# camillabelponer/dealii-slod

Measured on NVIDIA B200. Metric: slod_basis_patches_per_s, higher is better.
Workload: dtype f64

## Files before the change

dealii-slod_b200/csrc/capi.cu:

```cuda
#include <cuda_runtime.h>
#include <dlfcn.h>
#include <nccl.h>

#include <algorithm>
#include <array>
#include <cmath>
#include <cstdio>
#include <cstdlib>
#include <cstring>
#include <mutex>
#include <numeric>
#include <string>
#include <thread>
#include <vector>

#include "../../include/slod.h"
#include "geom.h"
#include "kernels.h"

using namespace slod;

namespace {

std::string g_create_error;

struct Timings {
  double ms[8] = {0, 0, 0, 0, 0, 0, 0, 0};
};

}

struct slod_ctx {
  slod_params par{};
  Params P{};
  int device = 0;
  int n_sm = 148;
  int64_t n_patches = 0;
  int n_fields = 1;
  bool coef_set[2] = {false, false};
  std::vector<double> coef_table[2];
  int coef_r[2] = {0, 0};
  bool coef_dirty = true;
  double *d_coef = nullptr;
  size_t d_coef_elems = 0;
  size_t coef_field_elems = 0;
  double *d_phi = nullptr, *d_aphi = nullptr, *d_Kell = nullptr, *d_diag = nullptr;
  int *d_status = nullptr;
  int *d_counter = nullptr;
  int *d_work_counter = nullptr;
  bool basis_done = false, coarse_done = false;
  int chunk = 0;
  bool chunk_limited = false;
  int64_t ids_cap = 0;
  int *d_ids = nullptr;
  double *d_X = nullptr, *d_Minv = nullptr, *d_G = nullptr, *d_cvec = nullptr, *d_Lws = nullptr, *d_W = nullptr, *d_coefws = nullptr;
  FluxLayout xl{};
  size_t smem_flux = 0;
  int grid_flux = 0;
  int solve_grid = 0;
  int dense_ntile = 0;
  int mma_variant = -1;
  bool dense_coef_gmem = false;
  int mma_threads = 0;
  int mma_nip = 0, mma_stw = 0;
  bool split_solver = false;
  size_t smem_factor = 0, smem_tri = 0;
  double *d_Lrec = nullptr;
  double *d_stw = nullptr;
  cudaEvent_t ev_split = nullptr;
  float split_factor_ms = 0;
  long long mma_lws_per_cta = 0;
  SolveLayout sl{};
  DenseLayout dl{};
  SelectPlan sp{};
  SelectBuffers sb{};
  FinishLayout fl{};
  size_t smem_solve = 0, smem_dense = 0, smem_finish = 0, smem_coarse = 0, smem_coarse_blk = 0;
  int coarse_nu = 0;
  int grid_solve = 0, grid_dense = 0, grid_finish = 0, grid_coarse = 0;
  int bw_max = 0, nb_max = 0;
  cudaEvent_t ev[12]{};
  std::vector<cudaEvent_t> chunk_ev;
  size_t chunks_pending = 0;
  bool basis_pending = false;
  int64_t pending_p0 = 0, pending_p1 = 0;
  int *h_status = nullptr;
  Timings tm;
  int64_t launches = 0;
  std::vector<int> ids;
  int64_t ids_p0 = -1, ids_p1 = -1;
  mutable std::string err;
  mutable std::vector<int64_t> fine_numbering;
  bool csr_ready = false;
  std::vector<int64_t> csr_rowptr, csr_col;
  long long *d_perm = nullptr;
  cudaStream_t copy_stream = nullptr;
  bool coarse_timing_pending = false;
  double *d_online = nullptr;
  size_t online_doubles = 0;
  double *d_batch = nullptr;
  size_t batch_doubles = 0;
  double *d_val = nullptr;
  int64_t csr_nnz = 0;
  double *d_Mell = nullptr, *d_Mval = nullptr, *d_Sell = nullptr;
  bool mass_done = false;
  double s_dt = 0.0;
  double *d_heat = nullptr;
  size_t heat_doubles = 0;
  std::vector<slod_ctx *> subs;
  ncclComm_t comm = nullptr;
  int comm_rank = 0, comm_world = 1;
// ... 432 lines not shown
  if (ctx->ids_p0 != p0 || ctx->ids_p1 != p1) {
    std::vector<int> order((size_t)(p1 - p0));
    std::iota(order.begin(), order.end(), (int)p0);
    std::vector<long long> cost(order.size());
    for (size_t i = 0; i < order.size(); ++i) {
      const Geom g = make_geom(P, order[i]);
      cost[i] = (long long)g.Ni * g.bw * (g.bw + 4LL * g.Ncd) + (long long)g.Ncd * g.Ncd * g.Ncd * 8;
    }
    std::vector<int> perm(order.size());
    std::iota(perm.begin(), perm.end(), 0);
    std::stable_sort(perm.begin(), perm.end(), [&](int a, int b) { return cost[a] > cost[b]; });
    ctx->ids.resize(order.size());
    for (size_t i = 0; i < perm.size(); ++i) ctx->ids[i] = order[perm[i]];
    CK(cudaMemcpyAsync(ctx->d_ids, ctx->ids.data(), sizeof(int) * ctx->ids.size(), cudaMemcpyHostToDevice, st));
    CK(cudaStreamSynchronize(st));
    ctx->ids_p0 = p0;
    ctx->ids_p1 = p1;
  }
  const size_t n_ids = ctx->ids.size();
  if (!ctx->h_status) CK(cudaHostAlloc(&ctx->h_status, sizeof(int) * (size_t)ctx->n_patches, cudaHostAllocDefault));
  CK(cudaMemsetAsync(ctx->d_status + p0, 0, sizeof(int) * (size_t)(p1 - p0), st));

  static const bool static_stride = getenv("SLOD_STATIC_WORK") != nullptr;
  int *wc = static_stride ? nullptr : ctx->d_work_counter;
  const size_t n_chunks = (n_ids + ctx->chunk - 1) / ctx->chunk;
  while (ctx->chunk_ev.size() < 5 * n_chunks) {
    cudaEvent_t e;
    CK(cudaEventCreate(&e));
    ctx->chunk_ev.push_back(e);
  }
  ctx->chunks_pending = 0;
  for (size_t off = 0, ci = 0; off < n_ids; off += ctx->chunk, ++ci) {
    const int nw = (int)std::min<size_t>(ctx->chunk, n_ids - off);
    const int *ids = ctx->d_ids + off;
    cudaEvent_t *ev = ctx->chunk_ev.data() + 5 * ci;
    CK(cudaEventRecord(ev[0], st));
    if (ctx->split_solver) {
      static const int factor_grid_env = getenv("SLOD_FACTOR_GRID") ? atoi(getenv("SLOD_FACTOR_GRID")) : 0;
      CK(launch_patch_factor(std::min(nw, factor_grid_env > 0 ? factor_grid_env : 2 * ctx->n_sm), ctx->smem_factor, st, ids, nw, ctx->d_coef, ctx->d_Lrec,
                             ctx->d_stw, ctx->d_status, ctx->sl.coef_doubles, ctx->mma_nip, ctx->sl.ldx, ctx->sl.x_stride, wc));
      if (ci == 0) CK(cudaEventRecord(ctx->ev_split, st));
      CK(launch_patch_trisolve(std::min(nw, ctx->n_sm), ctx->smem_tri, st, ids, nw, ctx->d_Lrec, ctx->d_X,
                               ctx->sl.coef_doubles, ctx->mma_nip, ctx->sl.ldx, ctx->sl.x_stride, wc));
      ctx->launches += 1;
    } else if (ctx->mma_variant >= 0)
      CK(launch_patch_solve_mma(ctx->mma_variant, std::min(nw, ctx->grid_solve), ctx->smem_solve, st, ids, nw,
                                ctx->d_coef, ctx->d_X, ctx->d_Lws, ctx->d_status, ctx->sl.coef_doubles, ctx->sl.ldx,
                                ctx->sl.x_stride, ctx->mma_lws_per_cta, ctx->mma_nip, ctx->mma_stw, wc));
    else
      CK(launch_patch_solve(std::min(nw, ctx->grid_solve), ctx->smem_solve, st, ids, nw, ctx->d_coef, ctx->d_X,
                            ctx->d_Lws, ctx->d_status, ctx->sl));
    CK(cudaEventRecord(ev[1], st));
    if (ctx->dense_ntile) {
      CK(launch_patch_flux(std::min(nw, ctx->grid_flux), ctx->smem_flux, st, ids, nw, ctx->d_coef, ctx->d_X,
                           ctx->d_W, ctx->xl, wc));
      CK(launch_patch_dense_mma(ctx->dense_ntile, std::min(nw, ctx->grid_dense), ctx->smem_dense, st, ids, nw,
                                ctx->d_coef, ctx->d_X, ctx->d_W, ctx->d_Minv, ctx->d_G, ctx->d_diag, ctx->d_status,
                                ctx->dl, wc));
      ctx->launches += 1;
    }
    else
      CK(launch_patch_dense(std::min(nw, ctx->grid_dense), ctx->smem_dense, st, ids, nw, ctx->d_coef, ctx->d_X,
                            ctx->d_Minv, ctx->d_G, ctx->d_diag, ctx->d_status, ctx->dl));
    CK(cudaEventRecord(ev[2], st));
    int nl = 0;
    CK(launch_select_pipeline(ctx->sp, st, ids, nw, ctx->d_Minv, ctx->d_G, ctx->d_cvec, ctx->d_diag,
                              ctx->d_status, ctx->sb, &nl));
    ctx->launches += nl;
    CK(cudaEventRecord(ev[3], st));
    CK(launch_patch_finish(std::min(nw, ctx->grid_finish), ctx->smem_finish, st, ids, nw, ctx->d_coef,
                           ctx->d_X, ctx->d_cvec, d_phi, d_aphi, ctx->fl));
    CK(cudaEventRecord(ev[4], st));
    ctx->launches += 3;
    ++ctx->chunks_pending;
  }
  CK(cudaMemcpyAsync(ctx->h_status + p0, ctx->d_status + p0, sizeof(int) * (size_t)(p1 - p0), cudaMemcpyDeviceToHost, st));
  CK(cudaEventRecord(ctx->ev[7], st));
  ctx->basis_pending = true;
  ctx->pending_p0 = p0;
  ctx->pending_p1 = p1;
  return SLOD_OK;
}

int wait_basis(slod_ctx *ctx) {
  if (!ctx->basis_pending) return SLOD_OK;
  ctx->basis_pending = false;
  CK(cudaEventSynchronize(ctx->ev[7]));
  float acc[4] = {0, 0, 0, 0};
  for (size_t ci = 0; ci < ctx->chunks_pending; ++ci)
    for (int k = 0; k < 4; ++k) {
      float ms = 0;
      CK(cudaEventElapsedTime(&ms, ctx->chunk_ev[5 * ci + k], ctx->chunk_ev[5 * ci + k + 1]));
      acc[k] += ms;
    }
  for (int k = 0; k < 4; ++k) ctx->tm.ms[k] = acc[k];
  if (ctx->split_solver && ctx->chunks_pending > 0) {
    float ms = 0;
    CK(cudaEventElapsedTime(&ms, ctx->chunk_ev[0], ctx->ev_split));
    ctx->tm.ms[5] = ms;
  }
  for (int64_t i = ctx->pending_p0; i < ctx->pending_p1; ++i)
    if (ctx->h_status[i]) {
      char buf[160];
      snprintf(buf, sizeof buf, "patch %lld: numerical status bits 0x%x (1 A_ii not SPD, 2 M not SPD, 4 Jacobi not converged)",
               (long long)i, ctx->h_status[i]);
      return fail(ctx, SLOD_ERR_NUMERIC, buf);
    }
  return SLOD_OK;
// ... 388 lines not shown
  SelectPlan &sp = ctx->sp;
  sp.s = P.s;
  sp.lay.threads = big ? 512 : 128;
  sp.lay.ncd_max = P.NcdMax; sp.lay.m_stride = dl.m_stride;
  sp.lay.fast_path = getenv("SLOD_NO_FAST_SELECT") ? 0 : 1;
  sp.smem_fast = select_fast_smem(P.NcdMax);
  sp.smem_jac = select_jacobi_smem(P.NcdMax);
  sp.eig.nmax = P.NcdMax; sp.eig.ldh = P.NcdMax;
  sp.eig.h_stride = (long long)P.NcdMax * P.NcdMax;
  sp.eig.v_stride = 6LL * P.NcdMax;
  sp.eig.log_cap = std::max<long long>(3LL * P.NcdMax * P.NcdMax, 1024);
  sp.eig.ncd_max = P.NcdMax; sp.eig.m_stride = dl.m_stride;
  sp.eig.cap_items = 0;
  sp.smem_tri = eig_tridiag_smem(P.NcdMax);
  sp.smem_ql = eig_ql_smem(P.NcdMax);
  sp.smem_fin = eig_finish_smem(P.NcdMax);
  sp.use_ql = (P.NcdMax - 1 <= 256 && sp.smem_tri <= prop.sharedMemPerBlockOptin && !getenv("SLOD_FORCE_JACOBI")) ? 1 : 0;
  FinishLayout &fl = ctx->fl;
  fl.ell_width = P.ell_width;
  fl.coef_doubles = coef_doubles; fl.nf_max = P.NfMax; fl.ncd_max = P.NcdMax; fl.ldx = sl.ldx; fl.x_stride = sl.x_stride;
  ctx->smem_finish = sizeof(double) * ((size_t)coef_doubles + P.NfMax + P.NcdMax) + sizeof(int) * ((size_t)P.NiMax + 2);
  ctx->smem_coarse = sizeof(double) * ((size_t)P.s * P.NfMax);
  const size_t smem_cap = prop.sharedMemPerBlockOptin;
  {
    const int nu = std::min((2 * P.ell + 2), P.N) * P.n + 1;
    const size_t sm = coarse_blocked_smem(P.dim, P.s, nu);
    if (P.ref >= 1 && sm + 2048 <= smem_cap && !getenv("SLOD_SIMPLE_COARSE")) {
      ctx->coarse_nu = nu;
      ctx->smem_coarse_blk = sm;
    }
  }
  if ((size_t)P.NcdMax * P.NcdMax > (size_t)32 * dl.threads)
    { delete ctx; return bad(SLOD_ERR_UNSUPPORTED, "patch too large: coarse dofs per patch exceed the Gram register tile"); }
  if (ctx->smem_solve > smem_cap || ctx->smem_dense > smem_cap || sp.smem_fast > smem_cap || sp.smem_jac > smem_cap ||
      ctx->smem_finish > smem_cap || ctx->smem_coarse > smem_cap) {
    delete ctx;
    return bad(SLOD_ERR_UNSUPPORTED, "patch too large for the shared-memory resident solver (oversampling/subdivisions)");
  }
  auto per_sm = [&](size_t smem, int threads) {
    int by_smem = (int)std::max<size_t>(1, (prop.sharedMemPerMultiprocessor) / (smem + 1024));
    int by_thr = std::max(1, 2048 / threads);
    return std::max(1, std::min(std::min(by_smem, by_thr), 16));
  };
  ctx->grid_solve = ctx->n_sm * per_sm(ctx->smem_solve, sl.threads);
  ctx->grid_dense = ctx->n_sm * per_sm(ctx->smem_dense, dl.threads);
  sp.grid_fast = ctx->n_sm * std::min(3, per_sm(sp.smem_fast, 256));
  sp.grid_jac = ctx->n_sm * per_sm(sp.smem_jac, sp.lay.threads);
  sp.grid_tri = ctx->n_sm * per_sm(sp.smem_tri, 256);
  sp.grid_fin = ctx->n_sm * per_sm(sp.smem_fin, 128);
  sp.grid_ql = ctx->n_sm * 8;
  ctx->grid_finish = ctx->n_sm * per_sm(ctx->smem_finish, 256);
  ctx->grid_flux = ctx->n_sm * std::min(getenv("SLOD_FLUX_CTAS") ? atoi(getenv("SLOD_FLUX_CTAS")) : 4, per_sm(ctx->smem_flux, 256));
  ctx->grid_coarse = ctx->n_sm * per_sm(ctx->smem_coarse, 256);

  auto cuda_bad = [&](const char *what, cudaError_t e) {
    g_create_error = std::string(what) + ": " + cudaGetErrorString(e);
    free_dev(ctx);
    delete ctx;
    return SLOD_ERR_CUDA;
  };
  cudaError_t e;
  ctx->coef_field_elems = (size_t)ipow(P.nsub, P.dim);
  if (maps_only) {
    *out = ctx;
    return SLOD_OK;
  }
  if ((e = cudaMalloc(&ctx->d_status, sizeof(int) * ctx->n_patches)) != cudaSuccess) return cuda_bad("cudaMalloc", e);
  if ((e = cudaMalloc(&ctx->d_diag, sizeof(double) * 8 * P.s * ctx->n_patches)) != cudaSuccess)
    return cuda_bad("cudaMalloc", e);
  cudaMemset(ctx->d_status, 0, sizeof(int) * ctx->n_patches);
  cudaMemset(ctx->d_diag, 0, sizeof(double) * 8 * P.s * ctx->n_patches);
  for (auto &ev : ctx->ev)
    if ((e = cudaEventCreate(&ev)) != cudaSuccess) return cuda_bad("cudaEventCreate", e);
  if ((e = cudaEventCreate(&ctx->ev_split)) != cudaSuccess) return cuda_bad("cudaEventCreate", e);
  if (par->n_gpus > 1) {
    NcclApi *nc = nccl_api();
    if (!nc->err.empty()) {
      g_create_error = nc->err;
      slod_destroy(ctx);
      return SLOD_ERR_CUDA;
    }
    const int N = par->n_gpus;
    slod_params sp1 = *par;
    sp1.n_gpus = 1;
    for (int r = 1; r < N; ++r) {
      sp1.device = dev + r;
      slod_ctx *sub = nullptr;
      const int rc = slod_create(&sp1, &sub);
      if (rc != SLOD_OK) {
        slod_destroy(ctx);
        return rc;
      }
      ctx->subs.push_back(sub);
    }
    std::vector<int> devs((size_t)N);
    for (int r = 0; r < N; ++r) devs[r] = dev + r;
    std::vector<ncclComm_t> comms((size_t)N);
    const ncclResult_t nr = nc->CommInitAll(comms.data(), N, devs.data());
    if (nr != ncclSuccess) {
      g_create_error = std::string("ncclCommInitAll: ") + nc->GetErrorString(nr);
      slod_destroy(ctx);
      return SLOD_ERR_CUDA;
    }
    for (int r = 0; r < N; ++r) {
      slod_ctx *c = rank_ctx(ctx, r);
      c->comm = comms[r];
// ... 1331 lines not shown
  *out = nullptr;
  return cudaHostAlloc(out, std::max<size_t>(bytes, 1), cudaHostAllocDefault) == cudaSuccess ? SLOD_OK : SLOD_ERR_CUDA;
}
int slod_free_host(void *p) {
  if (!p) return SLOD_OK;
  return cudaFreeHost(p) == cudaSuccess ? SLOD_OK : SLOD_ERR_CUDA;
}

int slod_ell_to_csr(const slod_ctx *ctx, const double *h_K, int64_t *rowptr, int64_t *col, double *val,
                    int64_t *n_rows, int64_t *nnz) {
  if (!ctx) return SLOD_ERR_INVALID;
  return ell_to_csr(ctx, h_K, rowptr, col, val, n_rows, nnz);
}

int slod_get_patch_diagnostics(const slod_ctx *ctx, int64_t patch, int comp, double out[8]) {
  int rc = check_patch(ctx, patch);
  if (rc) return rc;
  NEED_DEVICE();
  if (!out || comp < 0 || comp >= ctx->P.s) return fail(ctx, SLOD_ERR_INVALID, "bad argument");
  CK(cudaSetDevice(ctx->device));
  CK(cudaMemcpy(out, ctx->d_diag + ((size_t)patch * ctx->P.s + comp) * 8, sizeof(double) * 8, cudaMemcpyDeviceToHost));
  int st = 0;
  CK(cudaMemcpy(&st, ctx->d_status + patch, sizeof(int), cudaMemcpyDeviceToHost));
  out[7] = st;
  return SLOD_OK;
}

int slod_debug_patch_stages(slod_ctx *ctx, int64_t patch, double *X, double *Minv, double *G) {
  int rc = check_patch(ctx, patch);
  if (rc) return rc;
  NEED_DEVICE();
  CK(cudaSetDevice(ctx->device));
  rc = prepare_coefficients(ctx);
  if (rc) return rc;
  rc = wait_basis(ctx);
  if (rc) return rc;
  rc = ensure_workspace(ctx, 1);
  if (rc) return rc;
  BIND_PARAMS((cudaStream_t)0);
  ctx->ids_p0 = ctx->ids_p1 = -1;
  const int id = (int)patch;
  CK(cudaMemcpy(ctx->d_ids, &id, sizeof(int), cudaMemcpyHostToDevice));
  if (ctx->split_solver) {
    CK(launch_patch_factor(1, ctx->smem_factor, 0, ctx->d_ids, 1, ctx->d_coef, ctx->d_Lrec, ctx->d_stw, ctx->d_status,
                           ctx->sl.coef_doubles, ctx->mma_nip, ctx->sl.ldx, ctx->sl.x_stride, nullptr));
    CK(launch_patch_trisolve(1, ctx->smem_tri, 0, ctx->d_ids, 1, ctx->d_Lrec, ctx->d_X, ctx->sl.coef_doubles,
                             ctx->mma_nip, ctx->sl.ldx, ctx->sl.x_stride, nullptr));
  } else if (ctx->mma_variant >= 0)
    CK(launch_patch_solve_mma(ctx->mma_variant, 1, ctx->smem_solve, 0, ctx->d_ids, 1, ctx->d_coef, ctx->d_X, ctx->d_Lws,
                              ctx->d_status, ctx->sl.coef_doubles, ctx->sl.ldx, ctx->sl.x_stride, ctx->mma_lws_per_cta, ctx->mma_nip, ctx->mma_stw));
  else
    CK(launch_patch_solve(1, ctx->smem_solve, 0, ctx->d_ids, 1, ctx->d_coef, ctx->d_X, ctx->d_Lws, ctx->d_status, ctx->sl));
  if (ctx->dense_ntile) {
    CK(launch_patch_flux(1, ctx->smem_flux, 0, ctx->d_ids, 1, ctx->d_coef, ctx->d_X, ctx->d_W, ctx->xl));
    CK(launch_patch_dense_mma(ctx->dense_ntile, 1, ctx->smem_dense, 0, ctx->d_ids, 1, ctx->d_coef, ctx->d_X, ctx->d_W,
                              ctx->d_Minv, ctx->d_G, ctx->d_diag, ctx->d_status, ctx->dl));
  }
  else
    CK(launch_patch_dense(1, ctx->smem_dense, 0, ctx->d_ids, 1, ctx->d_coef, ctx->d_X, ctx->d_Minv, ctx->d_G, ctx->d_diag,
                          ctx->d_status, ctx->dl));
  ctx->launches += 2;
  CK(cudaDeviceSynchronize());
  const Geom g = make_geom(ctx->P, id);
  if (X) CK(cudaMemcpy2D(X, sizeof(double) * g.Ncd, ctx->d_X, sizeof(double) * ctx->sl.ldx, sizeof(double) * g.Ncd, g.Ni,
                         cudaMemcpyDeviceToHost));
  if (Minv) CK(cudaMemcpy(Minv, ctx->d_Minv, sizeof(double) * g.Ncd * g.Ncd, cudaMemcpyDeviceToHost));
  if (G) {
    if (!g.slod) return fail(ctx, SLOD_ERR_STATE, "patch takes the LOD branch: no Gram matrix");
    CK(cudaMemcpy(G, ctx->d_G, sizeof(double) * g.Ncd * g.Ncd, cudaMemcpyDeviceToHost));
  }
  if (ctx->split_solver) {
    std::vector<int> zpos((size_t)g.Ncd);
    for (int c = 0; c < g.Ncd; ++c) {
      int k[3];
      col_to_cell(ctx->P, g, c, k);
      zpos[c] = zcell_to_col(g, k);
    }
    std::vector<double> tmp;
    if (X) {
      tmp.assign(X, X + (size_t)g.Ni * g.Ncd);
      for (int r = 0; r < g.Ni; ++r)
        for (int c = 0; c < g.Ncd; ++c) X[(size_t)r * g.Ncd + c] = tmp[(size_t)r * g.Ncd + zpos[c]];
    }
    for (double *Mx : {Minv, G})
      if (Mx) {
        tmp.assign(Mx, Mx + (size_t)g.Ncd * g.Ncd);
        for (int r = 0; r < g.Ncd; ++r)
          for (int c = 0; c < g.Ncd; ++c) Mx[(size_t)r * g.Ncd + c] = tmp[(size_t)zpos[r] * g.Ncd + zpos[c]];
      }
  }
  return SLOD_OK;
}

int slod_measure_fp64_peak(slod_ctx *ctx, double *dfma_tflops, double *dmma_tflops) {
  if (!ctx || !dfma_tflops || !dmma_tflops) return SLOD_ERR_INVALID;
  NEED_DEVICE();
  CK(cudaSetDevice(ctx->device));
  CK(cudaDeviceSynchronize());
  CK(run_fp64_probe(ctx->n_sm, dfma_tflops, dmma_tflops));
  ctx->launches += 8;
  return SLOD_OK;
}

int slod_get_timings(const slod_ctx *ctx, double *ms, int n) {
  if (!ctx || !ms) return SLOD_ERR_INVALID;
  if (ctx->device != SLOD_DEVICE_NONE && (ctx->coarse_timing_pending || ctx->basis_pending)) {
    slod_ctx *c = const_cast<slod_ctx *>(ctx);
// ... 11 lines not shown
```

dealii-slod_b200/csrc/flux.cuh:

```cuda
#pragma once

namespace slod {

constexpr int kFTB = 64;
constexpr int kFNB = 20;

__global__ void __launch_bounds__(256, 4)
k_patch_flux(const int *__restrict__ patch_ids, int n_work, const double *__restrict__ d_coef,
             const double *__restrict__ Xbuf, double *__restrict__ Wbuf, FluxLayout lay, int *work_counter) {
  extern __shared__ double smem[];
  const int NC = lay.ldx;
  double *sCoef = smem;
  double *sArow = sCoef + lay.coef_doubles;
  int *sAnbr = (int *)(sArow + kFTB * kFNB);
  int *sAcnt = sAnbr + kFTB * kFNB;
  int *sBlist = sAcnt + kFTB;
  __shared__ int sNb;
  const int tid = threadIdx.x, NT = blockDim.x, lane = tid & 31, warp = tid >> 5, NWARP = NT >> 5;

  __shared__ int sNextWork;
  SLOD_WORK_LOOP(w, n_work, work_counter, sNextWork) {
    fetch_work_item(w, work_counter, &sNextWork);
    const Geom geo = make_geom(cP, patch_ids[w]);
    if (!geo.slod) continue;
// ... 83 lines not shown
#pragma unroll
          for (int u = 0; u < 4; ++u) {
            acc[u] = make_double2(0.0, 0.0);
            const int rb = r0 + u;
            if (rb < kFTB) cmax = max(cmax, sAcnt[rb]);
          }
          if (2 * c2 >= ncd) cmax = 0;
#pragma unroll 3
          for (int e = 0; e < cmax; ++e) {
#pragma unroll
            for (int u = 0; u < 4; ++u) {
              const int rb = min(r0 + u, kFTB - 1);
              const double av = sArow[rb * kFNB + e];
              const double2 xv = *reinterpret_cast<const double2 *>(X + (size_t)sAnbr[rb * kFNB + e] * lay.ldx + 2 * c2);
              acc[u].x += av * xv.x;
              acc[u].y += av * xv.y;
            }
          }
#pragma unroll
          for (int u = 0; u < 4; ++u) {
            const int rb = r0 + u;
            if (rb < kFTB && t0 + rb < nbd_pad)
              *reinterpret_cast<double2 *>(W + (size_t)(t0 + rb) * lay.ldx + 2 * c2) = acc[u];
          }
        }
      }
      __syncthreads();
      for (int idx = tid; idx < nt * 8; idx += NT) {
        const int rb = idx >> 3, corner = idx & 7;
        if (corner >= (1 << cP.dim)) continue;
        const int dof = sBlist[t0 + rb];
        int a[3];
        node_coords(geo, dof / s, a);
        int kc[3] = {0, 0, 0};
        double wgt = cP.pw;
        bool ok = true;
        _Pragma("unroll") for (int x = 0; x < 3; ++x) if (x < cP.dim) {
          const int q = a[x] >> lgn, rem = a[x] - (q << lgn);
          if ((corner >> x) & 1) {
            if (rem != 0 || q < 1) ok = false;
            kc[x] = q - 1;
          } else {
            if (q > geo.m[x] - 1) ok = false;
            kc[x] = q;
            if (rem != 0) wgt *= 2.0;
          }
        }
        if (ok) W[(size_t)(t0 + rb) * lay.ldx + (lay.zmajor ? zcell_to_col(geo, kc) : cell_to_col(cP, geo, kc)) * s + dof % s] -= wgt;
      }
    }
  }
}

}
```

dealii-slod_b200/csrc/kernels.cu:

```cuda
#include <cuda_runtime.h>
#include <math.h>
#include <stdint.h>
#include <stdio.h>
#include <stdlib.h>

#include "geom.h"
#include "kernels.h"

namespace slod {

__constant__ Params cP;

cudaError_t upload_params(const Params &p, cudaStream_t st) {
  return cudaMemcpyToSymbolAsync(cP, &p, sizeof(Params), 0, cudaMemcpyHostToDevice, st);
}

__device__ __forceinline__ int nfields() { return cP.problem == 0 ? 1 : 2; }

__device__ void load_coef(const Geom &g, const double *__restrict__ d_coef, double *sCoef, int t0 = -1, int nt = 0) {
  if (t0 < 0) { t0 = threadIdx.x; nt = blockDim.x; }
  const int n = cP.n;
  const int msx = g.m[0] * n, msy = g.m[1] * n, msz = (cP.dim == 3) ? g.m[2] * n : 1;
  const int nsubp = msx * msy * msz;
  const long long nsub = cP.nsub;
// ... 966 lines not shown
  return cudaGetLastError();
}

cudaError_t launch_patch_dense(int grid, size_t smem, cudaStream_t st, const int *ids, int n_work, const double *coef,
                               const double *X, double *Minv, double *G, double *diag, int *status,
                               const DenseLayout &lay) {
  cudaError_t e = cudaFuncSetAttribute(k_patch_dense, cudaFuncAttributeMaxDynamicSharedMemorySize, (int)smem);
  if (e != cudaSuccess) return e;
  k_patch_dense<<<grid, lay.threads, smem, st>>>(ids, n_work, coef, X, Minv, G, diag, status, lay);
  return cudaGetLastError();
}
template <int NTILE>
static cudaError_t launch_dense_t(int grid, size_t smem, cudaStream_t st, const int *ids, int n_work, const double *coef,
                                  const double *X, const double *W, double *Minv, double *G, double *diag, int *status,
                                  const DenseLayout &lay, int *work_counter) {
  cudaError_t e = cudaFuncSetAttribute(k_patch_dense_mma<NTILE>, cudaFuncAttributeMaxDynamicSharedMemorySize, (int)smem);
  if (e != cudaSuccess) return e;
  k_patch_dense_mma<NTILE><<<grid, 32 * NTILE, smem, st>>>(ids, n_work, coef, X, W, Minv, G, diag, status, lay, work_counter);
  return cudaGetLastError();
}
size_t dense_mma_smem(int ntile, int coef_doubles, int nb_max) {
  (void)nb_max;
  (void)coef_doubles;
  const int NC = 8 * ntile, LDM = NC + 4;
  return sizeof(double) * ((size_t)NC * LDM + 2 * (size_t)kDTB * LDM) + sizeof(int) * ((size_t)NC * 32 + 8);
}
cudaError_t launch_patch_dense_mma(int ntile, int grid, size_t smem, cudaStream_t st, const int *ids, int n_work,
                                   const double *coef, const double *X, const double *W, double *Minv, double *G,
                                   double *diag, int *status, const DenseLayout &lay, int *work_counter) {
  if (work_counter) {
    cudaError_t e = cudaMemsetAsync(work_counter, 0, sizeof(int), st);
    if (e != cudaSuccess) return e;
  }
  switch (ntile) {
    case 4: return launch_dense_t<4>(grid, smem, st, ids, n_work, coef, X, W, Minv, G, diag, status, lay, work_counter);
    case 8: return launch_dense_t<8>(grid, smem, st, ids, n_work, coef, X, W, Minv, G, diag, status, lay, work_counter);
    case 16: return launch_dense_t<16>(grid, smem, st, ids, n_work, coef, X, W, Minv, G, diag, status, lay, work_counter);
  }
  return cudaErrorInvalidValue;
}
size_t flux_smem(int coef_doubles, int ldx, int nb_max) {
  (void)ldx;
  return sizeof(double) * ((size_t)coef_doubles + (size_t)kFTB * kFNB) +
         sizeof(int) * ((size_t)kFTB * kFNB + kFTB + nb_max + 8);
}
cudaError_t launch_patch_flux(int grid, size_t smem, cudaStream_t st, const int *ids, int n_work, const double *coef,
                              const double *X, double *W, const FluxLayout &lay, int *work_counter) {
  cudaError_t e = cudaFuncSetAttribute(k_patch_flux, cudaFuncAttributeMaxDynamicSharedMemorySize, (int)smem);
  if (e != cudaSuccess) return e;
  if (work_counter && (e = cudaMemsetAsync(work_counter, 0, sizeof(int), st)) != cudaSuccess) return e;
  k_patch_flux<<<grid, 256, smem, st>>>(ids, n_work, coef, X, W, lay, work_counter);
  return cudaGetLastError();
}

size_t select_fast_smem(int ncd_max) {
  const size_t nbk = (size_t)(ncd_max + 6) / 8;
  return sizeof(double) * (nbk * (nbk + 1) / 2 * 64 + 8 * nbk + 8);
}
size_t select_jacobi_smem(int ncd_max) {
  return sizeof(double) * ((size_t)ncd_max * (ncd_max + 1) / 2 + (size_t)ncd_max * ncd_max + 6 * (size_t)ncd_max) +
         sizeof(int) * (3 * (size_t)ncd_max + 8);
}
size_t eig_tridiag_smem(int nmax) { return sizeof(double) * ((size_t)nmax * (nmax | 1) + 4 * (size_t)nmax); }
size_t eig_ql_smem(int nmax) { return sizeof(double) * 8 * 3 * (size_t)nmax; }
size_t eig_finish_smem(int nmax) {
  return sizeof(double) * ((size_t)nmax * kEigLd + 5 * (size_t)nmax) + sizeof(int) * ((size_t)nmax + 8);
}

cudaError_t launch_select_pipeline(const SelectPlan &pl, cudaStream_t st, const int *ids, int n_work, const double *Minv,
                                   const double *G, double *cvec, double *diag, int *status, const SelectBuffers &b,
                                   int *n_launches) {
  cudaError_t e;
#define SLOD_ATTR(k, sm)                                                                        \
  if ((e = cudaFuncSetAttribute(k, cudaFuncAttributeMaxDynamicSharedMemorySize, (int)(sm))) != cudaSuccess) return e
  SLOD_ATTR(k_select_fast, pl.smem_fast);
  SLOD_ATTR(k_select_jacobi, pl.smem_jac);
  if ((e = cudaMemsetAsync(b.counters, 0, 4 * sizeof(int), st)) != cudaSuccess) return e;
  k_select_fast<<<min(n_work, pl.grid_fast), 256, pl.smem_fast, st>>>(
      ids, n_work, Minv, G, cvec, diag, b.counters, pl.use_ql ? b.eig_list : b.jac_list, pl.use_ql ? 1 : 2, pl.lay);
  ++*n_launches;
  if (pl.use_ql) {
    SLOD_ATTR(k_eig_tridiag<4>, pl.smem_tri);
    SLOD_ATTR(k_eig_tridiag<8>, pl.smem_tri);
    SLOD_ATTR(k_eig_ql, pl.smem_ql);
    SLOD_ATTR(k_eig_finish, pl.smem_fin);
    const long long items_max = (long long)n_work * pl.s;
    for (long long off = 0; off < items_max; off += pl.eig.cap_items) {
      if (pl.eig.nmax - 1 <= 128)
        k_eig_tridiag<4><<<pl.grid_tri, 512, pl.smem_tri, st>>>(ids, b.counters, b.eig_list, (int)off, G, b.H, b.V, pl.eig);
      else
        k_eig_tridiag<8><<<pl.grid_tri, 512, pl.smem_tri, st>>>(ids, b.counters, b.eig_list, (int)off, G, b.H, b.V, pl.eig);
      k_eig_ql<<<pl.grid_ql, 256, pl.smem_ql, st>>>(ids, b.counters, b.eig_list, (int)off, b.V, b.rot_cs, b.rot_i,
                                                   b.rot_n, pl.eig);
      k_eig_finish<<<pl.grid_fin, 128, pl.smem_fin, st>>>(ids, b.counters, b.eig_list, (int)off, Minv, b.H, b.V,
                                                         b.rot_cs, b.rot_i, b.rot_n, cvec, diag, b.jac_list, pl.eig);
      *n_launches += 3;
    }
  }
  k_select_jacobi<<<pl.grid_jac, pl.lay.threads, pl.smem_jac, st>>>(ids, b.counters, b.jac_list, Minv, G, cvec, diag,
                                                                    status, pl.lay);
  ++*n_launches;
#undef SLOD_ATTR
  return cudaGetLastError();
}
cudaError_t launch_patch_finish(int grid, size_t smem, cudaStream_t st, const int *ids, int n_work, const double *coef,
                                const double *X, const double *cvec, double *phi, double *aphi,
// ... 253 lines not shown
```

dealii-slod_b200/csrc/kernels.h:

```cpp
#pragma once
#include <cuda_runtime.h>

#include "geom.h"

namespace slod {

constexpr int kSolveNB = 8;

struct SolveLayout {
  int threads;
  int R;
  int ldw;
  int ldr;
  int bw_max;
  int coef_doubles;
  int ldx;
  long long x_stride;
  long long lws_per_cta;
  int gmem_window;
  long long gwin_off;
};
struct DenseLayout {
  long long w_stride;
  int threads;
  int ncd_max, nb_max;
  int coef_doubles;
  int ldx;
  long long x_stride;
  long long m_stride;
  int zmajor;
  double *coef_ws;
};
struct FluxLayout {
  int coef_doubles;
  int ldx;
  int nb_max;
  long long x_stride;
  long long w_stride;
  int zmajor;
};
struct SelectLayout {
  int threads;
  int fast_path;
  int ncd_max;
  long long m_stride;
};
struct FinishLayout {
  int ell_width;
  int coef_doubles;
  int nf_max, ncd_max;
  int ldx;
  long long x_stride;
};

cudaError_t upload_params(const Params &p, cudaStream_t st);

cudaError_t launch_patch_solve(int grid, size_t smem, cudaStream_t st, const int *ids, int n_work, const double *coef,
                               double *X, double *Lws, int *status, const SolveLayout &lay);
size_t solve_mma_smem(int variant, int coef_doubles, int nip_max, int stw);
cudaError_t launch_patch_solve_mma(int variant, int grid, size_t smem, cudaStream_t st, const int *ids, int n_work,
                                   const double *coef, double *X, double *Lws, int *status, int coef_doubles, int ldx,
                                   long long x_stride, long long lws_per_cta, int nip_max, int stw,
                                   int *work_counter = nullptr);
size_t split_factor_smem(int coef_doubles, int nip_max);
size_t split_trisolve_smem(int nip_max);
long long split_rec_stride(int nip_max);
size_t split_stencil_ws_doubles(int grid, int nip_max);
cudaError_t launch_patch_factor(int grid, size_t smem, cudaStream_t st, const int *ids, int n_work, const double *coef,
                                double *Lrec, double *stencil_ws, int *status, int coef_doubles, int nip_max, int ldx,
                                long long x_stride, int *work_counter);
cudaError_t launch_patch_trisolve(int grid, size_t smem, cudaStream_t st, const int *ids, int n_work, const double *Lrec,
                                  double *X, int coef_doubles, int nip_max, int ldx, long long x_stride, int *work_counter);
cudaError_t launch_patch_dense(int grid, size_t smem, cudaStream_t st, const int *ids, int n_work, const double *coef,
                               const double *X, double *Minv, double *G, double *diag, int *status,
                               const DenseLayout &lay);
size_t flux_smem(int coef_doubles, int ldx, int nb_max);
cudaError_t launch_patch_flux(int grid, size_t smem, cudaStream_t st, const int *ids, int n_work, const double *coef,
                              const double *X, double *W, const FluxLayout &lay, int *work_counter = nullptr);
size_t dense_mma_smem(int ntile, int coef_doubles, int nb_max);
cudaError_t launch_patch_dense_mma(int ntile, int grid, size_t smem, cudaStream_t st, const int *ids, int n_work,
                                   const double *coef, const double *X, const double *W, double *Minv, double *G,
                                   double *diag, int *status, const DenseLayout &lay, int *work_counter = nullptr);
struct EigLayout {
  int nmax, ldh;
  long long h_stride, v_stride;
  long long log_cap;
  int ncd_max;
  long long m_stride;
  int cap_items;
};
struct SelectPlan {
  SelectLayout lay;
  EigLayout eig;
  int s;
  int use_ql;
  int grid_fast, grid_tri, grid_ql, grid_fin, grid_jac;
  size_t smem_fast, smem_tri, smem_ql, smem_fin, smem_jac;
};
struct SelectBuffers {
  int *counters;
  int *eig_list, *jac_list;
  double *H, *V;
  double2 *rot_cs;
  unsigned short *rot_i;
  int *rot_n;
};
size_t select_fast_smem(int ncd_max);
size_t select_jacobi_smem(int ncd_max);
size_t eig_tridiag_smem(int nmax);
size_t eig_ql_smem(int nmax);
size_t eig_finish_smem(int nmax);
cudaError_t launch_select_pipeline(const SelectPlan &pl, cudaStream_t st, const int *ids, int n_work, const double *Minv,
                                   const double *G, double *cvec, double *diag, int *status, const SelectBuffers &b,
                                   int *n_launches);
cudaError_t launch_patch_finish(int grid, size_t smem, cudaStream_t st, const int *ids, int n_work, const double *coef,
                                const double *X, const double *cvec, double *phi, double *aphi,
                                const FinishLayout &lay);
size_t coarse_blocked_smem(int dim, int s, int NU);
cudaError_t launch_coarse_blocked(int dim, int s, int grid, size_t smem, cudaStream_t st, int p0, int p1,
                                  const double *phi, const double *aphi, double *Kell, const FinishLayout &lay, int NU);
cudaError_t launch_gather(cudaStream_t st, const double *src, const long long *perm, double *dst, long long n);
cudaError_t launch_coarse_rhs(cudaStream_t st, int n_patches, int s, const double *phi, const double *f, double *b,
                              int nf_max);
cudaError_t launch_prolongate(cudaStream_t st, long long n_fine, const double *phi, const double *u, double *u_fine,
                              int nf_max);
enum FineOp {
  kFineStiffDirichlet = 0,
  kFineEnergy = 1,
  kFineMass = 2,
  kFineLaplace = 3,
  kFineHeatDirichlet = 4
// ... 38 lines not shown
```

Before: 220,700.

## Add staged flux kernel streaming X layers into a shared-memory ring via cp.async

```diff
diff --git a/dealii-slod_b200/csrc/capi.cu b/dealii-slod_b200/csrc/capi.cu
--- a/dealii-slod_b200/csrc/capi.cu
+++ b/dealii-slod_b200/csrc/capi.cu
@@ -57,6 +57,8 @@
   FluxLayout xl{};
   size_t smem_flux = 0;
   int grid_flux = 0;
+  size_t smem_flux_staged = 0;
+  int grid_flux_staged = 0;
   int solve_grid = 0;
   int dense_ntile = 0;
   int mma_variant = -1;
@@ -595,8 +597,8 @@
                             ctx->d_Lws, ctx->d_status, ctx->sl));
     CK(cudaEventRecord(ev[1], st));
     if (ctx->dense_ntile) {
-      CK(launch_patch_flux(std::min(nw, ctx->grid_flux), ctx->smem_flux, st, ids, nw, ctx->d_coef, ctx->d_X,
-                           ctx->d_W, ctx->xl, wc));
+      CK(launch_flux(ctx->grid_flux, ctx->smem_flux, ctx->grid_flux_staged, ctx->smem_flux_staged, st, ids, nw,
+                     ctx->d_coef, ctx->d_X, ctx->d_W, ctx->xl, wc));
       CK(launch_patch_dense_mma(ctx->dense_ntile, std::min(nw, ctx->grid_dense), ctx->smem_dense, st, ids, nw,
                                 ctx->d_coef, ctx->d_X, ctx->d_W, ctx->d_Minv, ctx->d_G, ctx->d_diag, ctx->d_status,
                                 ctx->dl, wc));
@@ -1091,6 +1093,29 @@
   ctx->grid_finish = ctx->n_sm * per_sm(ctx->smem_finish, 256);
   ctx->grid_flux = ctx->n_sm * std::min(getenv("SLOD_FLUX_CTAS") ? atoi(getenv("SLOD_FLUX_CTAS")) : 4, per_sm(ctx->smem_flux, 256));
   ctx->grid_coarse = ctx->n_sm * per_sm(ctx->smem_coarse, 256);
+  if (ctx->split_solver && P.dim == 3 && P.s == 1 && ctx->xl.zmajor && sl.ldx == 128 && !getenv("SLOD_FLUX_GATHER")) {
+    FluxLayout &xl = ctx->xl;
+    int need = 0;
+    for (int64_t pid = 0; pid < ctx->n_patches; ++pid) {
+      const Geom g = make_geom(P, (int)pid);
+      if (g.slod) need = std::max(need, flux_staged_min_rows(g));
+    }
+    xl.layer_rows_max = P.pmax * P.pmax;
+    xl.layer_cells_max = (P.pmax - 2) * (P.pmax - 2);
+    xl.arena_rows = need;
+    const size_t base = flux_staged_smem(xl);
+    const size_t per_cta = prop.sharedMemPerBlockOptin;
+    int rows = need;
+    if (base < per_cta) rows += (int)((per_cta - base) / (sl.ldx * sizeof(double)));
+    if (getenv("SLOD_FLUX_ARENA")) rows = std::max(need, atoi(getenv("SLOD_FLUX_ARENA")));
+    xl.arena_rows = rows;
+    const size_t sm = flux_staged_smem(xl);
+    if (need > 0 && sm <= prop.sharedMemPerBlockOptin) {
+      xl.staged = 1;
+      ctx->smem_flux_staged = sm;
+      ctx->grid_flux_staged = ctx->n_sm * per_sm(sm, 512);
+    }
+  }
 
   auto cuda_bad = [&](const char *what, cudaError_t e) {
     g_create_error = std::string(what) + ": " + cudaGetErrorString(e);
@@ -2528,7 +2553,8 @@
   else
     CK(launch_patch_solve(1, ctx->smem_solve, 0, ctx->d_ids, 1, ctx->d_coef, ctx->d_X, ctx->d_Lws, ctx->d_status, ctx->sl));
   if (ctx->dense_ntile) {
-    CK(launch_patch_flux(1, ctx->smem_flux, 0, ctx->d_ids, 1, ctx->d_coef, ctx->d_X, ctx->d_W, ctx->xl));
+    CK(launch_flux(1, ctx->smem_flux, 1, ctx->smem_flux_staged, 0, ctx->d_ids, 1, ctx->d_coef, ctx->d_X, ctx->d_W,
+                   ctx->xl));
     CK(launch_patch_dense_mma(ctx->dense_ntile, 1, ctx->smem_dense, 0, ctx->d_ids, 1, ctx->d_coef, ctx->d_X, ctx->d_W,
                               ctx->d_Minv, ctx->d_G, ctx->d_diag, ctx->d_status, ctx->dl));
   }
diff --git a/dealii-slod_b200/csrc/flux.cuh b/dealii-slod_b200/csrc/flux.cuh
--- a/dealii-slod_b200/csrc/flux.cuh
+++ b/dealii-slod_b200/csrc/flux.cuh
@@ -159,4 +159,316 @@
   }
 }
 
-}
+constexpr int kFSThreads = 512;
+constexpr int kFSHalf = 64;
+constexpr int kFSNB = 8;
+constexpr int kFSSeg = 6;
+constexpr int kFSVal = 10;
+
+struct FluxShape {
+  int p[3], q0, q1;
+  int sl0, sh0, sl1, sh1;
+  int flo, fhi;
+  int nperim;
+  int y0, len23;
+  int rowsP;
+  int rows0;
+  int nbd;
+};
+
+__host__ __device__ inline FluxShape flux_shape(const Geom &g) {
+  FluxShape f;
+  for (int a = 0; a < 3; ++a) f.p[a] = g.p[a];
+  f.q0 = g.p[0] - 2; f.q1 = g.p[1] - 2;
+  f.sl0 = !g.domlo[0]; f.sh0 = !g.domhi[0]; f.sl1 = !g.domlo[1]; f.sh1 = !g.domhi[1];
+  f.flo = !g.domlo[2]; f.fhi = !g.domhi[2];
+  f.nperim = 0;
+  for (int iy = 0; iy < f.q1; ++iy)
+    for (int ix = 0; ix < f.q0; ++ix)
+      f.nperim += ((ix == 0 && f.sl0) || (ix == f.q0 - 1 && f.sh0) || (iy == 0 && f.sl1) || (iy == f.q1 - 1 && f.sh1));
+  f.y0 = f.sl1 ? 1 : 0;
+  f.len23 = (f.sh1 ? g.p[1] - 2 : g.p[1] - 1) - f.y0 + 1;
+  f.rowsP = (f.sl1 + f.sh1) * g.p[0] + f.len23 * (f.sl0 + f.sh0);
+  f.rows0 = f.flo ? g.p[0] * g.p[1] : f.rowsP;
+  const int p2 = g.p[2];
+  f.nbd = f.rows0 + (p2 - 2) * f.rowsP + (f.fhi ? g.p[0] * g.p[1] : f.rowsP);
+  return f;
+}
+__host__ __device__ inline bool fs_full(const FluxShape &f, int j) { return (j == 1 && f.flo) || (j == f.p[2] - 2 && f.fhi); }
+__host__ __device__ inline int fs_cnt(const FluxShape &f, int j) { return fs_full(f, j) ? f.q0 * f.q1 : f.nperim; }
+__host__ __device__ inline int fs_start(const FluxShape &f, int j) {
+  return (j - 1) * f.nperim + ((j > 1 && fs_full(f, 1)) ? f.q0 * f.q1 - f.nperim : 0);
+}
+__host__ __device__ inline bool fs_face(const FluxShape &f, int k) { return (k == 0 && f.flo) || (k == f.p[2] - 1 && f.fhi); }
+__host__ __device__ inline int fs_rows(const FluxShape &f, int k) { return fs_face(f, k) ? f.p[0] * f.p[1] : f.rowsP; }
+__host__ __device__ inline int fs_wbase(const FluxShape &f, int k) { return k == 0 ? 0 : f.rows0 + (k - 1) * f.rowsP; }
+
+struct FluxLine {
+  int ax, cx, fx;
+  int t0, len, ext;
+  int rbase, rstep;
+  int a[3];
+  int ib, istep;
+  int across, cext;
+};
+__device__ __forceinline__ int fs_nlines(const FluxShape &f, int k) {
+  return fs_face(f, k) ? f.p[1] : f.sl1 + f.sh1 + f.sl0 + f.sh0;
+}
+__device__ __forceinline__ FluxLine fs_line(const FluxShape &f, int k, int li) {
+  FluxLine L;
+  L.a[2] = k;
+  if (fs_face(f, k)) {
+    L.ax = 0; L.cx = 1; L.fx = 2;
+    L.t0 = 0; L.len = f.p[0]; L.ext = f.p[0];
+    L.rbase = li * f.p[0]; L.rstep = 1;
+    L.a[0] = 0; L.a[1] = li;
+    L.ib = 0; L.istep = 1;
+    L.across = li; L.cext = f.p[1];
+    return L;
+  }
+  L.cx = 2; L.across = k; L.cext = f.p[2];
+  int which = li;
+  if (!f.sl1 && which >= 0) ++which;
+  if (!f.sh1 && which >= 1) ++which;
+  if (!f.sl0 && which >= 2) ++which;
+  const int mid = f.sl0 + f.sh0;
+  if (which <= 1) {
+    L.ax = 0; L.fx = 1;
+    L.t0 = 0; L.len = f.p[0]; L.ext = f.p[0];
+    L.rbase = (which == 0) ? 0 : (f.sl1 ? f.p[0] : 0) + f.len23 * mid;
+    L.rstep = 1;
+    L.a[0] = 0; L.a[1] = (which == 0) ? 0 : f.p[1] - 1;
+    L.ib = (which == 0) ? 0 : (f.q1 - 1) * f.q0; L.istep = 1;
+  } else {
+    L.ax = 1; L.fx = 0;
+    L.t0 = f.y0; L.len = f.len23; L.ext = f.p[1];
+    L.rbase = (f.sl1 ? f.p[0] : 0) + ((which == 3) ? f.sl0 : 0);
+    L.rstep = mid;
+    L.a[0] = (which == 2) ? 0 : f.p[0] - 1; L.a[1] = 0;
+    L.ib = (which == 2) ? 0 : f.q0 - 1; L.istep = f.q0;
+  }
+  return L;
+}
+
+__device__ __forceinline__ void cp_async16(void *dst, const void *src) {
+  asm volatile("cp.async.cg.shared.global [%0], [%1], 16;" ::"r"(smem_u32(dst)), "l"(src) : "memory");
+}
+__device__ __forceinline__ void cp_async_commit() { asm volatile("cp.async.commit_group;" ::: "memory"); }
+__device__ __forceinline__ void cp_async_wait_pending(int pending) {
+  switch (pending) {
+    case 0: asm volatile("cp.async.wait_group 0;" ::: "memory"); break;
+    case 1: asm volatile("cp.async.wait_group 1;" ::: "memory"); break;
+    case 2: asm volatile("cp.async.wait_group 2;" ::: "memory"); break;
+    case 3: asm volatile("cp.async.wait_group 3;" ::: "memory"); break;
+    case 4: asm volatile("cp.async.wait_group 4;" ::: "memory"); break;
+    case 5: asm volatile("cp.async.wait_group 5;" ::: "memory"); break;
+    case 6: asm volatile("cp.async.wait_group 6;" ::: "memory"); break;
+    default: asm volatile("cp.async.wait_group 7;" ::: "memory"); break;
+  }
+}
+
+__global__ void __launch_bounds__(kFSThreads, 1)
+k_patch_flux_staged(const int *__restrict__ patch_ids, int n_work, const double *__restrict__ d_coef,
+                    const double *__restrict__ Xbuf, double *__restrict__ Wbuf, FluxLayout lay, int *work_counter) {
+  extern __shared__ __align__(128) double smem[];
+  const int R = lay.arena_rows;
+  const int ldx = lay.ldx;
+  double *sArena = smem;
+  double *sVal = sArena + (size_t)R * ldx;
+  unsigned long long *sMask = (unsigned long long *)(sVal + (size_t)lay.layer_rows_max * kFSVal);
+  double *sCoef = (double *)(sMask + 2 * (size_t)lay.layer_rows_max);
+  int *sPos = (int *)(sCoef + lay.coef_doubles);
+  int *sList = sPos + lay.layer_cells_max;
+  __shared__ int sNextWork;
+  const int tid = threadIdx.x, lane = tid & 31, warp = tid >> 5;
+  const int h = warp >> 3, wh = warp & 7;
+  constexpr int NWH = kFSThreads / 64;
+  const int c2 = lane;
+  const int colA = kFSHalf * h + 2 * c2;
+  unsigned long long table_key = ~0ull;
+
+  SLOD_WORK_LOOP(w, n_work, work_counter, sNextWork) {
+    fetch_work_item(w, work_counter, &sNextWork);
+    const Geom geo = make_geom(cP, patch_ids[w]);
+    if (!geo.slod) continue;
+    const FluxShape f = flux_shape(geo);
+    const int ncd = geo.Ncd, p2 = f.p[2];
+    const int nbd_pad = (f.nbd + 31) & ~31;
+    const double *X = Xbuf + (size_t)w * lay.x_stride;
+    double *W = Wbuf + (size_t)w * lay.w_stride;
+    const bool live = colA < ncd;
+    __syncthreads();
+    const unsigned long long key = shape_key(geo);
+    if (key != table_key) {
+      table_key = key;
+      if (warp == 0) {
+        int count = 0;
+        for (int base = 0; base < f.q0 * f.q1; base += 32) {
+          const int idx = base + lane;
+          const int ix = idx % f.q0, iy = idx / f.q0;
+          const bool on = idx < f.q0 * f.q1 &&
+                          ((ix == 0 && f.sl0) || (ix == f.q0 - 1 && f.sh0) || (iy == 0 && f.sl1) || (iy == f.q1 - 1 && f.sh1));
+          const unsigned mask = __ballot_sync(0xffffffffu, on);
+          const int pos = count + __popc(mask & ((1u << lane) - 1u));
+          if (idx < f.q0 * f.q1) sPos[idx] = on ? pos : -1;
+          if (on) sList[pos] = idx;
+          count += __popc(mask);
+        }
+      }
+    }
+    load_coef(geo, d_coef, sCoef);
+    const int lgn = __ffs(cP.n) - 1;
+    __syncthreads();
+
+    int next = 1;
+    for (int k = 0; k < p2; ++k) {
+      {
+        const int keep = max(1, k - 1);
+        const int freed = fs_start(f, keep);
+        while (next <= p2 - 2 && fs_start(f, next) + fs_cnt(f, next) <= freed + R && next < keep + kFSNB) {
+          const int cnt = fs_cnt(f, next);
+          const bool full = fs_full(f, next);
+          const int st = fs_start(f, next) % R;
+          const double *Xl = X + (size_t)(next - 1) * f.q0 * f.q1 * ldx;
+          for (int e = tid; e < cnt * (ldx / 2); e += kFSThreads) {
+            const int i = e / (ldx / 2), part = e - i * (ldx / 2);
+            const int idx = full ? i : sList[i];
+            int r = st + i;
+            if (r >= R) r -= R;
+            cp_async16(sArena + (size_t)r * ldx + 2 * part, Xl + (size_t)idx * ldx + 2 * part);
+          }
+          cp_async_commit();
+          ++next;
+        }
+      }
+      const bool face = fs_face(f, k);
+      const int nl = fs_nlines(f, k);
+      const int lmax = max(f.p[0], f.p[1]);
+      for (int e = tid; e < nl * lmax * 10; e += kFSThreads) {
+        const int li = e / (lmax * 10), rem = e - li * lmax * 10, i = rem / 10, slot = rem - (rem / 10) * 10;
+        const FluxLine L = fs_line(f, k, li);
+        if (i >= L.len) continue;
+        const int c = L.t0 + i;
+        const int row = L.rbase + i * L.rstep;
+        int a[3];
+#pragma unroll
+        for (int x = 0; x < 3; ++x) a[x] = (x == L.ax) ? c : L.a[x];
+        if (slot == 9) {
+          double wgt = cP.pw;
+          unsigned long long m0 = 0, m1 = 0;
+#pragma unroll
+          for (int x = 0; x < 3; ++x) if ((a[x] & (cP.n - 1)) != 0) wgt *= 2.0;
+          for (int corner = 0; corner < 8; ++corner) {
+            int kc[3];
+            bool ok = true;
+#pragma unroll
+            for (int x = 0; x < 3; ++x) {
+              const int q = a[x] >> lgn, rm = a[x] - (q << lgn);
+              if ((corner >> x) & 1) { ok = ok && rm == 0 && q >= 1; kc[x] = q - 1; }
+              else { ok = ok && q <= geo.m[x] - 1; kc[x] = q; }
+            }
+            if (!ok) continue;
+            const int col = zcell_to_col(geo, kc);
+            if (col < 64) m0 |= 1ull << col;
+            else m1 |= 1ull << (col - 64);
+          }
+          sVal[(size_t)row * kFSVal + 9] = wgt;
+          sMask[2 * row] = m0;
+          sMask[2 * row + 1] = m1;
+          continue;
+        }
+        const int u = slot % 3 - 1, v = slot / 3 - 1;
+        int dl[3];
+#pragma unroll
+        for (int x = 0; x < 3; ++x) dl[x] = (x == L.ax) ? u : (x == L.cx) ? v : ((a[x] == 0) ? 1 : -1);
+        bool ok = true;
+#pragma unroll
+        for (int x = 0; x < 3; ++x) ok = ok && a[x] + dl[x] >= 1 && a[x] + dl[x] <= f.p[x] - 2;
+        sVal[(size_t)row * kFSVal + slot] = ok ? stiff_entry(cP, geo, sCoef, a, dl, 0, 0) : 0.0;
+      }
+      cp_async_wait_pending(next - 1 - min(p2 - 2, k + 1));
+      __syncthreads();
+      const int wbase = fs_wbase(f, k);
+      const int zf = (k == 0) ? 1 : p2 - 2;
+      int ntask = 0;
+      for (int li = 0; li < nl; ++li) ntask += (fs_line(f, k, li).len + kFSSeg - 1) / kFSSeg;
+      for (int task = wh; task < ntask; task += NWH) {
+        int li = 0, tt = task, nseg = 0;
+        FluxLine L;
+        for (;; ++li) {
+          L = fs_line(f, k, li);
+          nseg = (L.len + kFSSeg - 1) / kFSSeg;
+          if (tt < nseg) break;
+          tt -= nseg;
+        }
+        const int i0 = tt * kFSSeg, i1 = min(L.len, i0 + kFSSeg);
+        int lrow[3], lidx[3];
+        bool lfull[3];
+        const int vv = (L.across - 1 >= 1) ? 0 : (L.across >= 1 ? 1 : 2);
+#pragma unroll
+        for (int v = 0; v < 3; ++v) {
+          int cv = L.across + v - 1;
+          if (cv < 1 || cv > L.cext - 2) cv = L.across + vv - 1;
+          const int lz = face ? zf : cv;
+          lfull[v] = fs_full(f, lz);
+          lrow[v] = fs_start(f, lz) % R;
+          lidx[v] = L.ib + (face ? (cv - 1) * f.q0 : 0) - L.istep;
+        }
+        const double *colp = sArena + kFSHalf * h + 2 * c2;
+        auto ld = [&](int c, int v) -> double2 {
+          c = min(max(c, 1), L.ext - 2);
+          const int idx = lidx[v] + c * L.istep;
+          int r = lrow[v] + (lfull[v] ? idx : sPos[idx]);
+          if (r >= R) r -= R;
+          return *reinterpret_cast<const double2 *>(colp + (size_t)r * ldx);
+        };
+        double2 win[3][3];
+        if (live) {
+#pragma unroll
+          for (int v = 0; v < 3; ++v) {
+            win[v][1] = ld(L.t0 + i0 - 1, v);
+            win[v][2] = ld(L.t0 + i0, v);
+          }
+        }
+        for (int i = i0; i < i1; ++i) {
+          const int c = L.t0 + i;
+          const int r = L.rbase + i * L.rstep;
+          double2 acc = make_double2(0.0, 0.0);
+          if (live) {
+#pragma unroll
+            for (int v = 0; v < 3; ++v) {
+              win[v][0] = win[v][1];
+              win[v][1] = win[v][2];
+              win[v][2] = ld(c + 1, v);
+            }
+            const double2 *vp = reinterpret_cast<const double2 *>(sVal + (size_t)r * kFSVal);
+            double val[10];
+#pragma unroll
+            for (int t = 0; t < 5; ++t) {
+              const double2 d = vp[t];
+              val[2 * t] = d.x;
+              val[2 * t + 1] = d.y;
+            }
+#pragma unroll
+            for (int v = 0; v < 3; ++v)
+#pragma unroll
+              for (int u = 0; u < 3; ++u) {
+                acc.x = fma(val[3 * v + u], win[v][u].x, acc.x);
+                acc.y = fma(val[3 * v + u], win[v][u].y, acc.y);
+              }
+            const unsigned bits = (unsigned)(sMask[2 * r + h] >> (2 * c2)) & 3u;
+            if (bits & 1u) acc.x -= val[9];
+            if (bits & 2u) acc.y -= val[9];
+          }
+          *reinterpret_cast<double2 *>(W + (size_t)(wbase + r) * ldx + kFSHalf * h + 2 * c2) = acc;
+        }
+      }
+      __syncthreads();
+    }
+    for (int idx = tid; idx < (nbd_pad - f.nbd) * (ldx / 2); idx += kFSThreads)
+      *reinterpret_cast<double2 *>(W + (size_t)(f.nbd + idx / (ldx / 2)) * ldx + 2 * (idx % (ldx / 2))) =
+          make_double2(0.0, 0.0);
+  }
+}
+
+}
diff --git a/dealii-slod_b200/csrc/kernels.cu b/dealii-slod_b200/csrc/kernels.cu
--- a/dealii-slod_b200/csrc/kernels.cu
+++ b/dealii-slod_b200/csrc/kernels.cu
@@ -1042,6 +1042,36 @@
   k_patch_flux<<<grid, 256, smem, st>>>(ids, n_work, coef, X, W, lay, work_counter);
   return cudaGetLastError();
 }
+size_t flux_staged_smem(const FluxLayout &lay) {
+  return sizeof(double) * ((size_t)lay.arena_rows * lay.ldx + (size_t)lay.layer_rows_max * (kFSVal + 2) +
+                            lay.coef_doubles) +
+         sizeof(int) * 2 * (size_t)lay.layer_cells_max;
+}
+int flux_staged_min_rows(const Geom &g) {
+  const FluxShape f = flux_shape(g);
+  int need = 0;
+  for (int k = 0; k < g.p[2]; ++k) {
+    const int jlo = std::max(1, k - 1), jhi = std::min(g.p[2] - 2, k + 1);
+    need = std::max(need, fs_start(f, jhi) + fs_cnt(f, jhi) - fs_start(f, jlo));
+  }
+  return need;
+}
+cudaError_t launch_patch_flux_staged(int grid, size_t smem, cudaStream_t st, const int *ids, int n_work,
+                                     const double *coef, const double *X, double *W, const FluxLayout &lay,
+                                     int *work_counter) {
+  cudaError_t e = cudaFuncSetAttribute(k_patch_flux_staged, cudaFuncAttributeMaxDynamicSharedMemorySize, (int)smem);
+  if (e != cudaSuccess) return e;
+  if (work_counter && (e = cudaMemsetAsync(work_counter, 0, sizeof(int), st)) != cudaSuccess) return e;
+  k_patch_flux_staged<<<std::min(grid, n_work), kFSThreads, smem, st>>>(ids, n_work, coef, X, W, lay, work_counter);
+  return cudaGetLastError();
+}
+cudaError_t launch_flux(int grid_gather, size_t smem_gather, int grid_staged, size_t smem_staged, cudaStream_t st,
+                        const int *ids, int n_work, const double *coef, const double *X, double *W,
+                        const FluxLayout &lay, int *work_counter) {
+  if (lay.staged)
+    return launch_patch_flux_staged(grid_staged, smem_staged, st, ids, n_work, coef, X, W, lay, work_counter);
+  return launch_patch_flux(std::min(n_work, grid_gather), smem_gather, st, ids, n_work, coef, X, W, lay, work_counter);
+}
 
 size_t select_fast_smem(int ncd_max) {
   const size_t nbk = (size_t)(ncd_max + 6) / 8;
diff --git a/dealii-slod_b200/csrc/kernels.h b/dealii-slod_b200/csrc/kernels.h
--- a/dealii-slod_b200/csrc/kernels.h
+++ b/dealii-slod_b200/csrc/kernels.h
@@ -38,6 +38,10 @@
   long long x_stride;
   long long w_stride;
   int zmajor;
+  int staged;
+  int arena_rows;
+  int layer_rows_max;
+  int layer_cells_max;
 };
 struct SelectLayout {
   int threads;
@@ -77,6 +81,14 @@
 size_t flux_smem(int coef_doubles, int ldx, int nb_max);
 cudaError_t launch_patch_flux(int grid, size_t smem, cudaStream_t st, const int *ids, int n_work, const double *coef,
                               const double *X, double *W, const FluxLayout &lay, int *work_counter = nullptr);
+size_t flux_staged_smem(const FluxLayout &lay);
+int flux_staged_min_rows(const Geom &g);
+cudaError_t launch_patch_flux_staged(int grid, size_t smem, cudaStream_t st, const int *ids, int n_work,
+                                     const double *coef, const double *X, double *W, const FluxLayout &lay,
+                                     int *work_counter = nullptr);
+cudaError_t launch_flux(int grid_gather, size_t smem_gather, int grid_staged, size_t smem_staged, cudaStream_t st,
+                        const int *ids, int n_work, const double *coef, const double *X, double *W,
+                        const FluxLayout &lay, int *work_counter = nullptr);
 size_t dense_mma_smem(int ntile, int coef_doubles, int nb_max);
 cudaError_t launch_patch_dense_mma(int ntile, int grid, size_t smem, cudaStream_t st, const int *ids, int n_work,
                                    const double *coef, const double *X, const double *W, double *Minv, double *G,
```

New measurement: 211,200 (median of 6 runs). -4.3%, worse.
